# smups/rustronomy-watershed

Hardware: AMD Instinct MI355X
Metric: Mpixels/s segmenting watershed, 8192x8192 u8, device-resident (throughput, 4 transforms of distinct fields in flight; one transform alone: value_one_transform_alone) (higher is better)
Workload: dtype u8 image / u32 stamps+labels (integer min/max/compare); 1 GPU; 8192x8192 u8 uniform[0,254) random field per GPU, segmenting transform, max_water_level 254, seeds = find_local_minima (7320260 on rank 0's first field), engine fused; 4 contexts in flight, each transforming ITS OWN field and seed list (generator seeds 1..4); parallelism=independent fields x1, world_size=1, devices_visible=1, fields_per_gpu=1

## Files before the change

rustronomy-watershed_amd/csrc/ws_relax.hip:

```cpp
#include "ws_common.hpp"

#include <algorithm>
#include <cstdio>
#include <cstdlib>

namespace wsk {

typedef uint32_t u32x4_t __attribute__((ext_vector_type(4)));

#ifdef WS_DIAG_STAMPS
__device__ unsigned long long *g_diag = nullptr;
#define WS_STAMP(slot)                                                                          \
  do {                                                                                          \
    if (threadIdx.x == 0 && g_diag) g_diag[(size_t)blockIdx.x * 8 + (slot)] = __builtin_amdgcn_s_memrealtime(); \
  } while (0)
#define WS_STAMP_VALUE(slot, v)                                                                 \
  do {                                                                                          \
    if (threadIdx.x == 0 && g_diag) g_diag[(size_t)blockIdx.x * 8 + (slot)] = (v);              \
  } while (0)
#define WS_ACC_DECL unsigned long long ws_acc_t = 0, ws_acc[3] = {0, 0, 0}
#define WS_ACC_T0 (ws_acc_t = __builtin_amdgcn_s_memrealtime())
#define WS_ACC(k) do { const unsigned long long n_ = __builtin_amdgcn_s_memrealtime(); ws_acc[k] += n_ - ws_acc_t; ws_acc_t = n_; } while (0)
#define WS_ACC_STORE do { if (threadIdx.x == 0 && g_diag) { g_diag[(size_t)blockIdx.x * 8 + 5] = ws_acc[0]; g_diag[(size_t)blockIdx.x * 8 + 6] = ws_acc[1]; g_diag[(size_t)blockIdx.x * 8 + 7] = ws_acc[2]; } } while (0)
#else
// ... 1029 lines not shown
        run |= (st.x & ST_PASS) == pass || (st.y & ST_PASS) == pass || (st.z & ST_PASS) == pass || (st.w & ST_PASS) == pass;
      }
    run = run && tx * TW < W && ty * TH < H;
  }
  if ((uint32_t)t <= list_cap) tile_list[RL_HDR + 2 * (size_t)list_cap + t] = persist && run ? 1u : 0u;
  const unsigned long long todo = __builtin_amdgcn_ballot_w64(run);
  if (todo == 0) return;
  uint32_t base = 0;
  if (lane == 0) {
    base = atomicAdd(&tile_list[persist ? RLQ_TAIL : (pass & 3u)], (uint32_t)__popcll(todo));
    if (persist) atomicAdd(&tile_list[RLQ_PENDING], (uint32_t)__popcll(todo));
  }
  base = __shfl(base, 0, 64);
  const uint32_t idx = base + (uint32_t)__popcll(todo & ((1ull << lane) - 1ull));
  if (persist == 2) {
    uint32_t *avail = tile_list + pq_base(list_cap);
    if (lane == 0) atomicAdd(avail, (uint32_t)__popcll(todo));
    if ((lane & 31) == 0) (avail + PQ_HDR)[(first >> 5) + (lane >> 5)] = (uint32_t)(todo >> (lane & 32));
  } else if (run && persist) reinterpret_cast<unsigned long long *>(tile_list + RL_HDR)[idx] = ((unsigned long long)(idx + 1u) << 32) | (uint32_t)t;
  else if (run) tile_list[RL_HDR + (pass & 1u) * (size_t)list_cap + idx] = (uint32_t)t;
}

template <int TW, int TH>
__global__ __launch_bounds__(256) void k_relax_list_all(int H, int W, int tilesX, int tilesY, uint32_t pass, uint32_t *tile_list, uint32_t list_cap) {
  const int t = blockIdx.x * blockDim.x + threadIdx.x;
  if (t == 0) { tile_list[pass & 3u] = (uint32_t)(tilesX * tilesY); tile_list[4 + (pass & 3u)] = 0u; }
  if ((uint32_t)t <= list_cap) tile_list[RL_HDR + 2 * (size_t)list_cap + t] = 0u;
  if (t < tilesX * tilesY) tile_list[RL_HDR + (pass & 1u) * (size_t)list_cap + t] = (uint32_t)t;
}

size_t relax_list_words(int h, int w) {
  const uint32_t tiles = (uint32_t)relax_tiles(h, w);
  return pq_base(tiles) + PQ_HDR + (size_t)PQ_B * pq_words_per_bucket(tiles);
}

#ifndef WS_SPLIT_NW
#define WS_SPLIT_NW RX_NW
#endif
constexpr int RX_SNW = WS_SPLIT_NW;
constexpr int RX_STW = RX_TW / 2, RX_STH = 2 * RX_SNW * RX_P;
#ifndef WS_QUEUE_NW
#define WS_QUEUE_NW 16
#endif
constexpr int RX_QNW = WS_QUEUE_NW;
constexpr int RX_QTH = 2 * RX_QNW * RX_P;
size_t relax_tiles(int h, int w) {
  const int th = RX_NW * RX_P;
  const size_t a = (size_t)((w + RX_TW - 1) / RX_TW + 1) * ((h + th - 1) / th + 1);
  const size_t b = (size_t)((w + RX_STW - 1) / RX_STW + 1) * ((h + RX_STH - 1) / RX_STH + 1);
  return std::max(a, b);
}

__global__ void k_flag_tile_rows(uint32_t *prev, int sx, int bottom_row, uint32_t pass, int halo_flags) {
  const int i = blockIdx.x * blockDim.x + threadIdx.x;
  if (i >= sx * 4) return;
  if (halo_flags & 1) prev[i] = pass;
  if (halo_flags & 2) prev[(size_t)bottom_row * sx * 4 + i] = pass;
}

hipError_t block_flag_border_tiles(hipStream_t s, uint32_t *stamps, int h, int w, uint32_t pass, int halo_flags) {
  if ((pass & 1u) != 0 || h == 0 || w == 0) return hipErrorInvalidValue;
  const int th = RX_NW * RX_P;
  const int sx = (w + RX_TW - 1) / RX_TW + 1;
  const size_t cap = relax_tiles(h, w) * 4;
  const int bottom_row = (h - 2) / th + 1;
  k_flag_tile_rows<<<(sx * 4 + 255) / 256, 256, 0, s>>>(stamps + cap, sx, bottom_row, pass, halo_flags);
  return hipGetLastError();
}

constexpr int RX0_PH = 2 * RX_P;
constexpr int RX0_TH = RX_NW * RX0_PH;
typedef uint32_t tall_t[RX0_PH][RX_P];

template <bool TRACK, bool DOWN>
__device__ __forceinline__ void tall_sweep_rows(tall_t &T, const tall_t &B, const uint32_t (&up)[RX_P], const uint32_t (&dn)[RX_P],
                                                const uint32_t (&L)[RX0_PH], const uint32_t (&R)[RX0_PH], bool &changed) {
#pragma unroll
  for (int k = 0; k < RX0_PH; ++k) {
    const int r = DOWN ? k : RX0_PH - 1 - k;
#pragma unroll
    for (int c = 0; c < RX_P; ++c)
      relax_px<TRACK>(T[r][c], B[r][c], r == 0 ? up[c] : T[r - 1][c], r == RX0_PH - 1 ? dn[c] : T[r + 1][c],
                      c == 0 ? L[r] : T[r][c - 1], c == RX_P - 1 ? R[r] : T[r][c + 1], changed);
  }
}
template <bool TRACK, bool RIGHT>
__device__ __forceinline__ void tall_sweep_cols(tall_t &T, const tall_t &B, const uint32_t (&up)[RX_P], const uint32_t (&dn)[RX_P],
                                                const uint32_t (&L)[RX0_PH], const uint32_t (&R)[RX0_PH], bool &changed) {
#pragma unroll
  for (int k = 0; k < RX_P; ++k) {
    const int c = RIGHT ? k : RX_P - 1 - k;
#pragma unroll
    for (int r = 0; r < RX0_PH; ++r)
      relax_px<TRACK>(T[r][c], B[r][c], r == 0 ? up[c] : T[r - 1][c], r == RX0_PH - 1 ? dn[c] : T[r + 1][c],
                      c == 0 ? L[r] : T[r][c - 1], c == RX_P - 1 ? R[r] : T[r][c + 1], changed);
  }
}

__global__ __launch_bounds__(64 * RX_NW, 4) void k_relax0_tall(const uint8_t *__restrict__ img, uint32_t stride32, uint32_t *keys, int H, int W,
                                                               int tilesX, int flagAX, int flagSX, uint32_t max_level, uint32_t *stamps_own,
                                                               uint32_t *stamps_rerun, PassFlags pf, uint32_t max_iters,
                                                               const uint32_t *__restrict__ seed_mask, int SH, int check_carry, uint32_t *tile_list) {
  constexpr int NB = RX_NW, TW = RX_TW, TH = RX0_TH;
  constexpr uint32_t pass = 0;
  __shared__ __attribute__((aligned(16))) uint32_t sRow[2 * NB + 2][TW];
  __shared__ uint32_t s_flag[3];

  if (blockIdx.x == 0 && threadIdx.x < NSTRIPE)
    pf.edge_changed[((pass + 1) % COUNTER_RING) * FLAG_SLOT + threadIdx.x * STRIPE_STRIDE] = 0;
  if (tile_list && blockIdx.x == 0 && threadIdx.x == 0) { tile_list[(pass + 2) & 3u] = 0u; tile_list[4 + ((pass + 2) & 3u)] = 0u; }
  const int tile = (int)xcd_span_index(blockIdx.x, gridDim.x);
  const int tile_x = tile % tilesX, tile_y = tile / tilesX;
  const int x0 = tile_x * TW, y0 = tile_y * TH;
  if (x0 >= W || y0 >= H) return;
  const int tid = threadIdx.x, lane = tid & 63, band = tid >> 6;
  const int gx0 = x0 + lane * RX_P, gyb = y0 + band * RX0_PH;
  if (tid == 0) { s_flag[0] = 0; s_flag[1] = 0; s_flag[2] = 0; }

  tall_t T, B;
  uint32_t Lh[RX0_PH], Rh[RX0_PH];
  const bool dims24 = (uint32_t)W < (1u << 24) && (uint32_t)H < (1u << 24);
  const uint32_t gxc0 = (uint32_t)min(gx0, W - RX_P);
  const int xh_raw = lane < 32 ? x0 - 1 : x0 + TW;
  const uint32_t xh = (uint32_t)min(max(xh_raw, 0), W - 1);
  const bool xh_ok = lane < 32 ? x0 > 0 : x0 + TW < W;
  const int gy_halo_raw = band == 0 ? y0 - 1 : y0 + TH;
  const uint32_t gy_halo = (uint32_t)min(max(gy_halo_raw, 0), H - 1);
  u32x4_t halo_row;
  {
    uint32_t iv[RX0_PH];
#pragma unroll
    for (int r = 0; r < RX0_PH; ++r) {
      const uint32_t gyc = (uint32_t)min(gyb + r, H - 1);
      const uint32_t ro = dims24 ? __umul24(gyc, (uint32_t)W) : gyc * (uint32_t)W;
      const uint32_t p = ro + gxc0, ph_ = ro + xh;
      const uint32_t nib = seed_mask[p >> 5] >> (p & 31u);
      iv[r] = *reinterpret_cast<const uint32_t *>(img + ((unsigned long long)gyc * stride32 + gxc0));
      Lh[r] = (seed_mask[ph_ >> 5] >> (ph_ & 31u)) & 1u;
      T[r][0] = nib & 1u; T[r][1] = nib & 2u; T[r][2] = nib & 4u; T[r][3] = nib & 8u;
    }
    const uint32_t p = (dims24 ? __umul24(gy_halo, (uint32_t)W) : gy_halo * (uint32_t)W) + gxc0;
    const uint32_t nib = seed_mask[p >> 5] >> (p & 31u);
    halo_row = u32x4_t{nib & 1u, nib & 2u, nib & 4u, nib & 8u};
    if (max_level == 254u) {
#pragma unroll
      for (int r = 0; r < RX0_PH; ++r) {
        B[r][0] = (iv[r] << 24) | 1u;
        B[r][1] = ((iv[r] << 16) & 0xFF000000u) | 1u;
        B[r][2] = ((iv[r] << 8) & 0xFF000000u) | 1u;
        B[r][3] = (iv[r] & 0xFF000000u) | 1u;
      }
    } else {
#pragma unroll
      for (int r = 0; r < RX0_PH; ++r)
#pragma unroll
        for (int c = 0; c < RX_P; ++c) {
          const uint32_t v = (iv[r] >> (8 * c)) & 0xFFu;
          B[r][c] = v <= max_level ? ((v << 24) | 1u) : KEY_INF;
        }
    }
  }
#pragma unroll
  for (int r = 0; r < RX0_PH; ++r) {
#pragma unroll
    for (int c = 0; c < RX_P; ++c) T[r][c] = T[r][c] ? 0u : KEY_INF;
    Lh[r] = Lh[r] ? 0u : KEY_INF;
  }
  halo_row.x = halo_row.x ? 0u : KEY_INF; halo_row.y = halo_row.y ? 0u : KEY_INF;
  halo_row.z = halo_row.z ? 0u : KEY_INF; halo_row.w = halo_row.w ? 0u : KEY_INF;
  const bool inner = SH == H && x0 >= 1 && x0 + TW <= W - 1 && y0 >= 1 && y0 + TH <= H - 1;
  if (!inner) {
    int ry = SH == H ? gyb : gyb % SH;
#pragma unroll
    for (int r = 0; r < RX0_PH; ++r) {
      const int gy = gyb + r;
      const bool row_ok = gy < H, row_int = ry >= 1 && ry < SH - 1 && gy < H;
#pragma unroll
      for (int c = 0; c < RX_P; ++c) {
        const int gx = gx0 + c;
        if (!(row_ok && gx < W)) T[r][c] = KEY_INF;
        if (!(row_int && gx >= 1 && gx < W - 1)) B[r][c] = KEY_INF;
      }
      if (!(row_ok && xh_ok)) Lh[r] = KEY_INF;
      if (++ry == SH) ry = 0;
    }
    const bool ok = gy_halo_raw >= 0 && gy_halo_raw < H;
    if (!(ok && gx0 + 0 < W)) halo_row.x = KEY_INF;
    if (!(ok && gx0 + 1 < W)) halo_row.y = KEY_INF;
    if (!(ok && gx0 + 2 < W)) halo_row.z = KEY_INF;
    if (!(ok && gx0 + 3 < W)) halo_row.w = KEY_INF;
  }
#pragma unroll
  for (int r = 0; r < RX0_PH; ++r) {
#pragma unroll
    for (int c = 0; c < RX_P; ++c) B[r][c] = min(B[r][c], T[r][c]);
    Rh[r] = Lh[r];
  }
  auto refresh_columns = [&]() {
#pragma unroll
    for (int r = 0; r < RX0_PH; ++r) {
      Lh[r] = lane_left(Lh[r], T[r][3]);
      Rh[r] = lane_right(Rh[r], T[r][0]);
    }
  };
  auto publish_rows = [&]() {
    *reinterpret_cast<u32x4_t *>(&sRow[1 + 2 * band][lane * RX_P]) = u32x4_t{T[0][0], T[0][1], T[0][2], T[0][3]};
    *reinterpret_cast<u32x4_t *>(&sRow[2 + 2 * band][lane * RX_P]) = u32x4_t{T[RX0_PH - 1][0], T[RX0_PH - 1][1], T[RX0_PH - 1][2], T[RX0_PH - 1][3]};
  };
  if (band == 0) *reinterpret_cast<u32x4_t *>(&sRow[0][lane * RX_P]) = halo_row;
  if (band == NB - 1) *reinterpret_cast<u32x4_t *>(&sRow[2 * NB + 1][lane * RX_P]) = halo_row;
  publish_rows();
  __syncthreads();

  uint32_t iters = 0;
  bool unfinished = max_iters == 0;
  uint32_t up[RX_P], dn[RX_P];
  auto fetch_rows = [&]() {
    const u32x4_t up4 = *reinterpret_cast<const u32x4_t *>(&sRow[2 * band][lane * RX_P]);
    const u32x4_t dn4 = *reinterpret_cast<const u32x4_t *>(&sRow[2 * band + 3][lane * RX_P]);
    up[0] = up4.x; up[1] = up4.y; up[2] = up4.z; up[3] = up4.w;
    dn[0] = dn4.x; dn[1] = dn4.y; dn[2] = dn4.z; dn[3] = dn4.w;
  };
  for (; max_iters != 0;) {
    ++iters;
    if (iters <= 2) {
      bool untracked = false;
      fetch_rows();
      refresh_columns();
      tall_sweep_rows<false, true>(T, B, up, dn, Lh, Rh, untracked);
      refresh_columns();
      tall_sweep_cols<false, true>(T, B, up, dn, Lh, Rh, untracked);
      refresh_columns();
      tall_sweep_rows<false, false>(T, B, up, dn, Lh, Rh, untracked);
      publish_rows();
      __syncthreads();
    }
    bool changed = false;
    fetch_rows();
    refresh_columns();
    tall_sweep_cols<true, false>(T, B, up, dn, Lh, Rh, changed);
    const uint32_t slot = (iters - 1) % 3;
    if (__builtin_amdgcn_ballot_w64(changed) != 0) {
      publish_rows();
      if (lane == 0) s_flag[slot] = 1;
    }
    __syncthreads();
    const bool again = s_flag[slot] != 0;
    if (tid == 0) s_flag[(slot + 2) % 3] = 0;
    if (!again) break;
    if (iters >= max_iters) { unfinished = true; break; }
  }

  uint32_t ovf = 0;
  if (gx0 < W) {
#pragma unroll
    for (int r = 0; r < RX0_PH; ++r) {
      const int gy = gyb + r;
      if (gy < H) *reinterpret_cast<u32x4_t *>(keys + (size_t)gy * W + gx0) = u32x4_t{T[r][0], T[r][1], T[r][2], T[r][3]};
      if (check_carry) {
#pragma unroll
        for (int c = 0; c < RX_P; ++c)
          ovf |= (T[r][c] != 0u && T[r][c] < KEY_INF && (T[r][c] & RING_MASK) == 0u);
      }
    }
  }
  if (ovf) atomicExch(pf.overflow, 1u);
  const uint32_t stripe = (blockIdx.x % NSTRIPE) * STRIPE_STRIDE;
  auto matters = [](uint32_t now, uint32_t across) { return now != 0u && now + 1u < across; };
  bool edge = false;
  if (band == 0) {
    const u32x4_t a = *reinterpret_cast<const u32x4_t *>(&sRow[0][lane * RX_P]);
    edge |= matters(T[0][0], a.x) || matters(T[0][1], a.y) || matters(T[0][2], a.z) || matters(T[0][3], a.w);
  }
  if (band == NB - 1) {
    const u32x4_t a = *reinterpret_cast<const u32x4_t *>(&sRow[2 * NB + 1][lane * RX_P]);
    constexpr int l = RX0_PH - 1;
    edge |= matters(T[l][0], a.x) || matters(T[l][1], a.y) || matters(T[l][2], a.z) || matters(T[l][3], a.w);
  }
  if (lane == 0 || lane == 63) {
#pragma unroll
    for (int r = 0; r < RX0_PH; ++r) edge |= matters(T[r][lane == 0 ? 0 : 3], lane == 0 ? Lh[r] : Rh[r]);
  }
  if (edge) pf.edge_changed[(pass % COUNTER_RING) * FLAG_SLOT + stripe] = 1u;
  if (tid == 0) {
    if (unfinished) {
#pragma unroll
      for (int k = 0; k < RX0_TH / (RX_NW * RX_P); ++k) {
        const int fy = tile_y * (RX0_TH / (RX_NW * RX_P)) + k;
        if (fy * (RX_NW * RX_P) >= H) break;
        stamps_rerun[((size_t)fy * flagSX + tile_x + 1) * 4 + 2] = pass + 2;
        uint32_t *own = stamps_own + ((size_t)fy * flagAX + tile_x) * 4;
        own[0] = pass + 1; own[1] = pass + 1; own[2] = pass + 1; own[3] = pass + 1;
      }
      pf.edge_changed[(pass % COUNTER_RING) * FLAG_SLOT + stripe] = 1u;
    }
    pf.any_change[stripe] = 1u;
    if (pf.stats) {
      atomicAdd(&pf.stats[stripe], (uint32_t)(TW * TH / 2048));
      atomicAdd(&pf.stats[FLAG_SLOT + stripe], 2u * iters);
    }
  }
}

bool relax_uses_seam_repair(int h, int w, bool seed_bits, int slice_h, bool padded, size_t seam_min_px) {
  const int ax = (w + RX_TW - 1) / RX_TW, ay = (h + RX_NW * RX_P - 1) / (RX_NW * RX_P);
  (void)slice_h;
  return seed_bits && !padded && (w & 3) == 0 && ax >= 2 && ay >= 2 && (size_t)h * (size_t)w >= seam_min_px;
}

hipError_t relax_pass(hipStream_t s, const uint8_t *img, size_t img_stride, uint32_t *keys, int h, int w,
                      uint32_t max_level, uint32_t pass, uint32_t *stamps, PassFlags pf, uint32_t max_iters,
                      const uint32_t *seed_labels, bool seed_bits, int slice_h, bool carry_checked_later, bool padded,
                      uint32_t *tile_list, size_t seam_min_px, int persistent_pass) {
  const int th = RX_NW * RX_P;
  const int pad = padded ? 1 : 0;
  const int check_carry = carry_checked_later ? 0 : 1;
  const int sh = slice_h > 0 ? slice_h : h;
  const int ax = (w + RX_TW - 1) / RX_TW, ay = (h + th - 1) / th;
  const int sx = ax + 1, sy = ay + 1;
  static const uint32_t same_from_passes = [] {
    const char *e = tuning_env("WS_RELAX_SAME_GRID_FROM");
    const uint32_t v = e ? (uint32_t)atoi(e) : RX_SAME_GRID_FROM;
    return v < 3u ? 3u : (v | 1u);
  }();
  static const uint32_t queue_from = [] {
    const char *e = tuning_env("WS_RELAX_QUEUE_FROM");
    const uint32_t v = e ? (uint32_t)atoi(e) : 3u;
    return v < 3u ? 3u : (v | 1u);
  }();
  const int persist_mode = tuning_env("WS_RELAX_PERSIST") ? atoi(tuning_env("WS_RELAX_PERSIST")) : persistent_pass;
  const bool queue_plane = persist_mode == 2 && tile_list && !pad && (w & 3) == 0 && w >= RX_P &&
                           ((reinterpret_cast<uintptr_t>(img) | img_stride) & 3u) == 0 && relax_tiles(h, w) < (1u << 24);
  const bool early_queue = (queue_plane || (persist_mode == 4 && tile_list)) && queue_from < same_from_passes;
  const uint32_t same_from = early_queue ? queue_from : same_from_passes;
  const int read_same = pass >= same_from ? 1 : 0, write_same = pass + 1 >= same_from ? 1 : 0;
  const uint32_t list_cap = (uint32_t)relax_tiles(h, w);
  const int shifted = read_same ? 0 : (int)(pass & 1u);
  const int tx = shifted ? sx : ax, ty = shifted ? sy : ay;
  const size_t cap = relax_tiles(h, w) * 4;
  const uint32_t *prev = stamps + ((pass + 1) & 1) * cap;
  uint32_t *cur = stamps + (pass & 1) * cap;
  const int ox_ = read_same ? ax : (shifted ? ax : sx), oy_ = read_same ? ay : (shifted ? ay : sy);
  static const uint32_t p0_rounds = [] {
    const char *e = tuning_env("WS_RELAX_P0_ROUNDS");
    return e ? (uint32_t)atoi(e) : 2u;
  }();
  static const bool no_seam = tuning_env("WS_RELAX_NO_SEAM") != nullptr;
  const bool seam_flow = !no_seam && seed_labels != nullptr && relax_uses_seam_repair(h, w, seed_bits, slice_h, padded, seam_min_px);
  constexpr uint32_t SEAM_P0_ROUNDS = 6;
  const uint32_t p0_cap = seam_flow ? SEAM_P0_ROUNDS : p0_rounds;
  if (pass == 0 && p0_cap < max_iters) max_iters = p0_cap;
  static const uint32_t late_cap = [] {
    const char *e = tuning_env("WS_RELAX_LATE_CAP");
    return e ? (uint32_t)atoi(e) : RX_LATE_ROUND_CAP;
  }();
  static const uint32_t scan_from_knob = [] {
    const char *e = tuning_env("WS_RELAX_SCAN_FROM");
    return e ? (uint32_t)atoi(e) : RX_SCAN_FROM_PASS;
  }();
  const uint32_t scan_from = early_queue ? same_from - 1u : std::max(scan_from_knob, 1u);
  if (pass >= scan_from && late_cap != 0 && late_cap < max_iters) max_iters = late_cap;
  if (const char *e = tuning_env("WS_RELAX_WIDE_CAP")) {
    int n_ = 0, c_ = 0;
    if (sscanf(e, "%d,%d", &n_, &c_) == 2 && pass >= scan_from && pass < scan_from + (uint32_t)n_) max_iters = (uint32_t)c_;
  }
  static const uint32_t early_cap = [] {
    const char *e = tuning_env("WS_RELAX_EARLY_CAP");
    return e ? (uint32_t)atoi(e) : RX_EARLY_ROUND_CAP;
  }();
  if (pass >= 1 && pass < scan_from && early_cap != 0 && early_cap < max_iters) max_iters = early_cap;
  static const uint32_t lite_from = [] {
    const char *e = tuning_env("WS_RELAX_LITE_FROM");
    return e ? (uint32_t)atoi(e) : 2u;
  }();
  static const uint32_t chunk_from = [] {
    const char *e = tuning_env("WS_RELAX_CHUNK_FROM");
    return e ? (uint32_t)atoi(e) : 3u;
  }();
  constexpr uint32_t SEAM_REPAIR_ROUNDS = 4;
  static const int seam_band = [] { const char *e = tuning_env("WS_RELAX_SEAM_BAND"); return e ? atoi(e) : 6; }();
  static const bool no_tall = tuning_env("WS_RELAX_NO_TALL") != nullptr;
  const bool tall0 = seam_flow && !no_tall && seam_band == 6 && h > RX0_TH && w >= RX_P &&
                     ((reinterpret_cast<uintptr_t>(img) | img_stride) & 3u) == 0 && img_stride <= 0xFFFFFFFFull;
  const int ay_tall = (h + RX0_TH - 1) / RX0_TH;
  if (tall0 && pass == 0) {
    k_relax0_tall<<<ax * ay_tall, 64 * RX_NW, 0, s>>>(img, (uint32_t)img_stride, keys, h, w, ax, ax, sx, max_level, cur, const_cast<uint32_t *>(prev), pf,
                                                     max_iters, seed_labels, sh, check_carry, tile_list);
    return hipGetLastError();
  }
  if (tall0 && pass == 1) {
    k_relax<3, false, false, false, false, 1, 0, RX0_TH><<<ax * (ay_tall - 1), 192, 0, s>>>(img, img_stride, keys, h, w, ax, ay_tall - 1, sx, sy, 0, 1, max_level, pass, prev, cur,
                                                                                          pf, SEAM_REPAIR_ROUNDS, nullptr, 0, sh, check_carry, pad, tile_list, 0, 0, 0, list_cap, 0);
  } else if (seam_flow && pass == 1) {
    if (seam_band == 4)
      k_relax<2, false, false, false, false, 1><<<ax * (ay - 1), 128, 0, s>>>(img, img_stride, keys, h, w, ax, ay - 1, sx, sy, 0, 1, max_level, pass, prev, cur,
                                                                            pf, SEAM_REPAIR_ROUNDS, nullptr, 0, sh, check_carry, pad, tile_list, 0, 0, 0, list_cap, 0);
    else if (seam_band == 6)
      k_relax<3, false, false, false, false, 1><<<ax * (ay - 1), 192, 0, s>>>(img, img_stride, keys, h, w, ax, ay - 1, sx, sy, 0, 1, max_level, pass, prev, cur,
                                                                            pf, SEAM_REPAIR_ROUNDS, nullptr, 0, sh, check_carry, pad, tile_list, 0, 0, 0, list_cap, 0);
    else
      k_relax<4, false, false, false, false, 1><<<ax * (ay - 1), 256, 0, s>>>(img, img_stride, keys, h, w, ax, ay - 1, sx, sy, 0, 1, max_level, pass, prev, cur,
                                                                            pf, SEAM_REPAIR_ROUNDS, nullptr, 0, sh, check_carry, pad, tile_list, 0, 0, 0, list_cap, 0);
  }
  if (seam_flow && pass == 1) {
    hipError_t e = hipGetLastError();
    if (e != hipSuccess) return e;
    const int strips_x = (ax - 1 + 31) / 32;
    k_relax<RX_NW, false, false, false, false, 2><<<strips_x * ay, 64 * RX_NW, 0, s>>>(img, img_stride, keys, h, w, strips_x, ay, sx, sy, 0, 1, max_level, pass,
                                                                                       prev, cur, pf, SEAM_REPAIR_ROUNDS, nullptr, 0, sh, check_carry, pad, tile_list, 0, 0,
                                                                                       0, list_cap, 0);
    return hipGetLastError();
  }
  const int sb = pass == 0 && seed_labels && seed_bits ? 1 : 0;
  const uint32_t *sl = pass == 0 ? seed_labels : nullptr;
  const uint32_t chunk_from_now = seam_flow ? std::min(chunk_from, 2u) : chunk_from;
  if (pass < chunk_from_now && pass < lite_from) {
    k_relax<RX_NW, false, false, false><<<tx * ty, 64 * RX_NW, 0, s>>>(img, img_stride, keys, h, w, tx, ty, ox_, oy_, shifted, seam_flow && pass == 0 ? 3 : 1, max_level, pass,
                                                                       prev, cur, pf, max_iters, sl, sb, sh, check_carry, pad, tile_list, 0, read_same, write_same, list_cap, 0);
  } else if (pass < chunk_from_now) {
    k_relax<RX_NW, false, false, true><<<tx * ty, 64 * RX_NW, 0, s>>>(img, img_stride, keys, h, w, tx, ty, ox_, oy_, shifted, 1, max_level, pass,
                                                                      prev, cur, pf, max_iters, sl, sb, sh, check_carry, pad, tile_list, 0, read_same, write_same, list_cap, 0);
  } else {
    const int chunk = 4;
    const unsigned grid = (unsigned)((tx * ty + chunk - 1) / chunk);
    static const uint32_t list_from_passes = [] {
      const char *e = tuning_env("WS_RELAX_LIST_FROM");
      return e ? (uint32_t)atoi(e) : RX_LIST_FROM_PASS;
    }();
    const uint32_t list_from = early_queue ? same_from : list_from_passes;
    if (pass < scan_from) {
      k_relax<RX_NW, true, false, true><<<grid, 64 * RX_NW, 0, s>>>(img, img_stride, keys, h, w, tx, ty, ox_, oy_, shifted, chunk, max_level,
                                                              pass, prev, cur, pf, max_iters, nullptr, 0, sh, check_carry, pad, tile_list, 0, read_same, write_same, list_cap, 0);
    } else if (tile_list && pass >= list_from && pass >= scan_from + 1) {
      static const bool no_append = tuning_env("WS_RELAX_NO_APPEND") != nullptr;
      const uint32_t first_list_pass = std::max(list_from, scan_from + 1);
      const int append_next = !no_append && pass >= same_from && pass >= first_list_pass ? 1 : 0;
      const bool appended = !no_append && pass >= 1 && pass - 1 >= same_from && pass - 1 >= first_list_pass;
      static const bool no_split = tuning_env("WS_RELAX_NO_SPLIT") != nullptr;
      const bool split = !no_split && pass >= same_from && same_from >= first_list_pass;
      const int gx = split ? (w + RX_STW - 1) / RX_STW : tx, gy = split ? (h + RX_STH - 1) / RX_STH : ty;
      if (!appended) {
        const unsigned blocks = (unsigned)((std::max<size_t>((size_t)gx * gy, list_cap + 1) + 255) / 256);
        const bool persist = (persist_mode == 1 || persist_mode == 2) && split && pass == same_from && !pad && (w & 3) == 0 && w >= RX_P &&
                             ((reinterpret_cast<uintptr_t>(img) | img_stride) & 3u) == 0 && (size_t)gx * gy <= list_cap && list_cap < (1u << 24);
        if (persist) {
          const bool in_order = persist_mode == 2;
          hipError_t e = hipMemsetAsync(tile_list + RL_HDR, 0, 2 * (size_t)list_cap * sizeof(uint32_t), s);
          if (e == hipSuccess) e = hipMemsetAsync(tile_list + 8, 0, (RL_HDR - 8) * sizeof(uint32_t), s);
          if (e == hipSuccess && in_order)
            e = hipMemsetAsync(tile_list + pq_base(list_cap), 0, (PQ_HDR + (size_t)PQ_B * pq_words_per_bucket(list_cap)) * sizeof(uint32_t), s);
          if (e != hipSuccess) return e;
          const int qy = (h + RX_QTH - 1) / RX_QTH;
          if (in_order)
            k_relax_list_regrid<RX_STW, RX_QTH, RX_TW, RX_NW * RX_P><<<blocks, 256, 0, s>>>(h, w, gx, qy, ax, ay, pass, prev, tile_list, list_cap, 2);
          else
            k_relax_list_regrid<RX_STW, RX_STH, RX_TW, RX_NW * RX_P><<<blocks, 256, 0, s>>>(h, w, gx, gy, ax, ay, pass, prev, tile_list, list_cap, 1);
          if ((e = hipGetLastError()) != hipSuccess) return e;
          const unsigned workers = tuning_env("WS_RELAX_PERSIST_WORKERS") ? (unsigned)atoi(tuning_env("WS_RELAX_PERSIST_WORKERS"))
                                                                          : std::min<unsigned>(in_order ? RX_LIST_GRID / 2 : RX_LIST_GRID * RX_NW / RX_SNW, (unsigned)(gx * (in_order ? qy : gy)));
          const uint32_t cap = tuning_env("WS_RELAX_PERSIST_CAP") ? (uint32_t)atoi(tuning_env("WS_RELAX_PERSIST_CAP")) : RLQ_ROUND_CAP;
          const int mode = tuning_env("WS_RELAX_PERSIST_MODE") ? atoi(tuning_env("WS_RELAX_PERSIST_MODE")) : 0;
          if (in_order)
            k_relax<RX_QNW, true, true, true, true, 0, 2><<<workers, 64 * RX_QNW, 0, s>>>(img, img_stride, keys, h, w, gx, qy, gx, qy, 0, chunk, max_level, pass, prev, cur, pf, cap,
                                                                                         nullptr, 0, sh, check_carry, pad, tile_list, mode, 1, 1, list_cap, 1);
          else
            k_relax<RX_SNW, true, true, true, true, 0, 1><<<workers, 64 * RX_SNW, 0, s>>>(img, img_stride, keys, h, w, gx, gy, gx, gy, 0, chunk, max_level, pass, prev, cur, pf, cap,
                                                                                         nullptr, 0, sh, check_carry, pad, tile_list, mode, 1, 1, list_cap, 1);
          if ((e = hipGetLastError()) != hipSuccess) return e;
          hipStreamCaptureStatus capturing = hipStreamCaptureStatusNone;
          (void)hipStreamIsCapturing(s, &capturing);
          if (tuning_env("WS_RELAX_PERSIST_DIAG") && capturing == hipStreamCaptureStatusNone) {
            uint32_t hd[RL_HDR];
            (void)hipStreamSynchronize(s);
            (void)hipMemcpy(hd, tile_list, sizeof hd, hipMemcpyDeviceToHost);
            fprintf(stderr, "[ws] persistent pass %u: pushed %u popped %u pending %u done %u runs %u | workers wait %.1f us, life %.1f us (sums / 512), polls %u\n", pass,
                    hd[RLQ_TAIL], hd[RLQ_HEAD], hd[RLQ_PENDING], hd[RLQ_DONE], hd[RLQ_RUNS], hd[RLQ_WAIT] / 100.0 / 512.0, hd[RLQ_LIFE] / 100.0 / 512.0, hd[RLQ_POLLS]);
            const double runs = hd[RLQ_RUNS] ? hd[RLQ_RUNS] : 1;
            fprintf(stderr, "[ws]   per tile run (us): load %.2f rounds %.2f epilogue %.2f hand-in %.2f; shader clock %.0f MHz\n", hd[RLQ_PHASE] / 100.0 / runs, hd[RLQ_PHASE + 1] / 100.0 / runs,
                    hd[RLQ_PHASE + 2] / 100.0 / runs, hd[RLQ_PHASE + 3] / 100.0 / runs, hd[RLQ_LIFE] ? 256.0 * hd[RLQ_PHASE + 4] / hd[RLQ_LIFE] * 100.0 : 0.0);
          }
          k_relax_list_all<RX_STW, RX_STH><<<(unsigned)((std::max<size_t>((size_t)gx * gy, list_cap + 1) + 255) / 256), 256, 0, s>>>(h, w, gx, gy, pass + 1, tile_list, list_cap);
          return hipGetLastError();
        }
        if (split && pass == same_from)
          k_relax_list_regrid<RX_STW, RX_STH, RX_TW, RX_NW * RX_P><<<blocks, 256, 0, s>>>(h, w, gx, gy, ax, ay, pass, prev, tile_list, list_cap, 0);
        else if (split)
          k_relax_list<RX_STW, RX_STH><<<blocks, 256, 0, s>>>(h, w, gx, gy, gx, gy, 0, pass, prev, tile_list, 1, list_cap);
        else
          k_relax_list<RX_TW, RX_NW * RX_P><<<blocks, 256, 0, s>>>(h, w, tx, ty, ox_, oy_, shifted, pass, prev, tile_list, read_same, list_cap);
        hipError_t e = hipGetLastError();
        if (e != hipSuccess) return e;
      }
      if (split)
        k_relax<RX_SNW, true, true, true, true><<<std::min<unsigned>(RX_LIST_GRID * RX_NW / RX_SNW, (unsigned)(gx * gy)), 64 * RX_SNW, 0, s>>>(
            img, img_stride, keys, h, w, gx, gy, gx, gy, 0, chunk, max_level, pass, prev, cur, pf, max_iters, nullptr, 0, sh,
            check_carry, pad, tile_list, 1, 1, 1, list_cap, append_next);
      else
        k_relax<RX_NW, true, true, true><<<std::min<unsigned>(RX_LIST_GRID, (unsigned)(tx * ty)), 64 * RX_NW, 0, s>>>(
            img, img_stride, keys, h, w, tx, ty, ox_, oy_, shifted, chunk, max_level, pass, prev, cur, pf, max_iters, nullptr, 0, sh,
            check_carry, pad, tile_list, 1, read_same, write_same, list_cap, append_next);
    } else {
      k_relax<RX_NW, true, true, true><<<grid, 64 * RX_NW, 0, s>>>(img, img_stride, keys, h, w, tx, ty, ox_, oy_, shifted, chunk, max_level,
                                                             pass, prev, cur, pf, max_iters, nullptr, 0, sh, check_carry, pad, tile_list, 0, read_same, write_same, list_cap, 0);
    }
  }
  return hipGetLastError();
}

}
```

Before: 160,300 Mpixels/s.

## Add tall-tile vertical seam strip relaxation kernel for pass one

Adds a specialized kernel that relaxes the vertical seams between column tiles using tall tiles (RX0_TH rows) held in registers, with DPP lane exchange for horizontal neighbours and shared-memory row exchange between bands. It replaces the generic strip kernel when the tall pass-0 layout is active, covering each seam with fewer, taller blocks. Blocks whose seam stamps are already settled exit early, and stamp marking follows the tall-tile geometry. It adds a new code path with its own boundary and stamp logic, which can be disabled through an environment variable.

```diff
diff --git a/rustronomy-watershed_amd/csrc/ws_relax.hip b/rustronomy-watershed_amd/csrc/ws_relax.hip
--- a/rustronomy-watershed_amd/csrc/ws_relax.hip
+++ b/rustronomy-watershed_amd/csrc/ws_relax.hip
@@ -1355,6 +1355,239 @@
   }
 }
 
+__global__ __launch_bounds__(64 * RX_NW, 4) void k_relax_strips_tall(const uint8_t *__restrict__ img, uint32_t stride32, uint32_t *keys, int H, int W,
+                                                                     int stripsX, int flagSX, uint32_t max_level, uint32_t pass, uint32_t *stamps_cur,
+                                                                     PassFlags pf, uint32_t max_iters, int SH, int check_carry, uint32_t *tile_list) {
+  constexpr int NB = RX_NW, TW = RX_TW, TH = RX0_TH;
+  constexpr int SEAM_PY = RX_NW * RX_P, SEAM_PX = RX_TW;
+  __shared__ __attribute__((aligned(16))) uint32_t sRow[2 * NB + 2][TW];
+  __shared__ __attribute__((aligned(16))) uint32_t sInitRow[2][TW];
+  __shared__ uint32_t s_flag[3];
+  __shared__ uint32_t s_edges;
+  __shared__ uint64_t s_sum[64 * NB];
+  __shared__ uint32_t sInitCol[RX0_PH][64 * NB];
+
+  if (blockIdx.x == 0 && threadIdx.x < NSTRIPE)
+    pf.edge_changed[((pass + 1) % COUNTER_RING) * FLAG_SLOT + threadIdx.x * STRIPE_STRIDE] = 0;
+  if (tile_list && blockIdx.x == 0 && threadIdx.x == 0) { tile_list[(pass + 2) & 3u] = 0u; tile_list[4 + ((pass + 2) & 3u)] = 0u; }
+  const int tile = (int)xcd_span_index(blockIdx.x, gridDim.x);
+  const int tile_x = tile % stripsX, tile_y = tile / stripsX;
+  const int y0 = tile_y * TH;
+  if (y0 >= H || (tile_x * 32 + 1) * SEAM_PX >= W) return;
+  const int tid = threadIdx.x, lane = tid & 63, band = tid >> 6;
+  const int seam_x = (tile_x * 32 + (lane >> 1) + 1) * SEAM_PX;
+  const bool has_seam = seam_x < W;
+  const int fx = seam_x / SEAM_PX - 1 + (lane & 1);
+  {
+    bool settled = true;
+#pragma unroll
+    for (int k = 0; k < TH / SEAM_PY; ++k) {
+      const int fy = tile_y * (TH / SEAM_PY) + k;
+      const bool there = has_seam && fy * SEAM_PY < H;
+      const uint32_t word = stamps_cur[there ? ((size_t)fy * flagSX + fx + 1) * 4 + 2 : 2];
+      settled &= !there || word == pass + 1;
+    }
+    if (__builtin_amdgcn_ballot_w64(settled) == ~0ull) return;
+  }
+  const int gx0 = has_seam ? seam_x - RX_P + (lane & 1) * RX_P : W, gyb = y0 + band * RX0_PH;
+  if (tid == 0) { s_edges = 0; s_flag[0] = 0; s_flag[1] = 0; s_flag[2] = 0; }
+
+  tall_t T, B;
+  uint32_t halo[RX0_PH];
+  const uint32_t gxc0 = (uint32_t)min(gx0, W - RX_P);
+  const int xh_raw = (lane & 1) ? gx0 + RX_P : gx0 - 1;
+  const uint32_t xh = (uint32_t)min(max(xh_raw, 0), W - 1);
+  const bool xh_ok = has_seam && xh_raw < W;
+  const int gy_halo_raw = band == 0 ? y0 - 1 : y0 + TH;
+  const uint32_t gy_halo = (uint32_t)min(max(gy_halo_raw, 0), H - 1);
+  u32x4_t halo_row;
+  {
+    u32x4_t kv[RX0_PH];
+    uint32_t iv[RX0_PH];
+#pragma unroll
+    for (int r = 0; r < RX0_PH; ++r) {
+      const uint32_t gyc = (uint32_t)min(gyb + r, H - 1);
+      iv[r] = *reinterpret_cast<const uint32_t *>(img + ((unsigned long long)gyc * stride32 + gxc0));
+      kv[r] = *reinterpret_cast<const u32x4_t *>(keys + (size_t)gyc * W + gxc0);
+      halo[r] = keys[(size_t)gyc * W + xh];
+    }
+    halo_row = *reinterpret_cast<const u32x4_t *>(keys + (size_t)gy_halo * W + gxc0);
+#pragma unroll
+    for (int r = 0; r < RX0_PH; ++r) { T[r][0] = kv[r].x; T[r][1] = kv[r].y; T[r][2] = kv[r].z; T[r][3] = kv[r].w; }
+    if (max_level == 254u) {
+#pragma unroll
+      for (int r = 0; r < RX0_PH; ++r) {
+        B[r][0] = (iv[r] << 24) | 1u;
+        B[r][1] = ((iv[r] << 16) & 0xFF000000u) | 1u;
+        B[r][2] = ((iv[r] << 8) & 0xFF000000u) | 1u;
+        B[r][3] = (iv[r] & 0xFF000000u) | 1u;
+      }
+    } else {
+#pragma unroll
+      for (int r = 0; r < RX0_PH; ++r)
+#pragma unroll
+        for (int c = 0; c < RX_P; ++c) {
+          const uint32_t v = (iv[r] >> (8 * c)) & 0xFFu;
+          B[r][c] = v <= max_level ? ((v << 24) | 1u) : KEY_INF;
+        }
+    }
+  }
+  {
+    int ry = SH == H ? gyb : gyb % SH;
+#pragma unroll
+    for (int r = 0; r < RX0_PH; ++r) {
+      const int gy = gyb + r;
+      const bool row_ok = gy < H, row_int = ry >= 1 && ry < SH - 1 && gy < H;
+#pragma unroll
+      for (int c = 0; c < RX_P; ++c) {
+        const int gx = gx0 + c;
+        if (!(row_ok && gx < W)) T[r][c] = KEY_INF;
+        if (!(row_int && gx >= 1 && gx < W - 1)) B[r][c] = KEY_INF;
+      }
+      if (!(row_ok && xh_ok)) halo[r] = KEY_INF;
+      if (++ry == SH) ry = 0;
+    }
+    const bool ok = gy_halo_raw >= 0 && gy_halo_raw < H;
+    if (!(ok && gx0 + 0 < W)) halo_row.x = KEY_INF;
+    if (!(ok && gx0 + 1 < W)) halo_row.y = KEY_INF;
+    if (!(ok && gx0 + 2 < W)) halo_row.z = KEY_INF;
+    if (!(ok && gx0 + 3 < W)) halo_row.w = KEY_INF;
+  }
+  uint32_t Lh[RX0_PH], Rh[RX0_PH];
+  {
+    uint64_t sum_before = 0;
+#pragma unroll
+    for (int r = 0; r < RX0_PH; ++r) {
+#pragma unroll
+      for (int c = 0; c < RX_P; ++c) {
+        B[r][c] = min(B[r][c], T[r][c]);
+        sum_before += T[r][c];
+      }
+      Lh[r] = halo[r];
+      Rh[r] = halo[r];
+      sInitCol[r][tid] = (lane & 1) ? T[r][RX_P - 1] : T[r][0];
+    }
+    s_sum[tid] = sum_before;
+  }
+  auto refresh_columns = [&]() {
+#pragma unroll
+    for (int r = 0; r < RX0_PH; ++r) {
+      Lh[r] = lane_left(Lh[r], T[r][RX_P - 1]);
+      Rh[r] = lane_right(Rh[r], T[r][0]);
+      Lh[r] = (lane & 1) ? Lh[r] : halo[r];
+      Rh[r] = (lane & 1) ? halo[r] : Rh[r];
+    }
+  };
+  auto publish_rows = [&]() {
+    *reinterpret_cast<u32x4_t *>(&sRow[1 + 2 * band][lane * RX_P]) = u32x4_t{T[0][0], T[0][1], T[0][2], T[0][3]};
+    *reinterpret_cast<u32x4_t *>(&sRow[2 + 2 * band][lane * RX_P]) = u32x4_t{T[RX0_PH - 1][0], T[RX0_PH - 1][1], T[RX0_PH - 1][2], T[RX0_PH - 1][3]};
+  };
+  if (band == 0) {
+    *reinterpret_cast<u32x4_t *>(&sRow[0][lane * RX_P]) = halo_row;
+    *reinterpret_cast<u32x4_t *>(&sInitRow[0][lane * RX_P]) = u32x4_t{T[0][0], T[0][1], T[0][2], T[0][3]};
+  }
+  if (band == NB - 1) {
+    *reinterpret_cast<u32x4_t *>(&sRow[2 * NB + 1][lane * RX_P]) = halo_row;
+    *reinterpret_cast<u32x4_t *>(&sInitRow[1][lane * RX_P]) = u32x4_t{T[RX0_PH - 1][0], T[RX0_PH - 1][1], T[RX0_PH - 1][2], T[RX0_PH - 1][3]};
+  }
+  publish_rows();
+  __syncthreads();
+
+  uint32_t iters = 0;
+  bool unfinished = max_iters == 0;
+  uint32_t up[RX_P], dn[RX_P];
+  auto fetch_rows = [&]() {
+    const u32x4_t up4 = *reinterpret_cast<const u32x4_t *>(&sRow[2 * band][lane * RX_P]);
+    const u32x4_t dn4 = *reinterpret_cast<const u32x4_t *>(&sRow[2 * band + 3][lane * RX_P]);
+    up[0] = up4.x; up[1] = up4.y; up[2] = up4.z; up[3] = up4.w;
+    dn[0] = dn4.x; dn[1] = dn4.y; dn[2] = dn4.z; dn[3] = dn4.w;
+  };
+  for (; max_iters != 0;) {
+    ++iters;
+    {
+      bool untracked = false;
+      fetch_rows();
+      refresh_columns();
+      tall_sweep_rows<false, true>(T, B, up, dn, Lh, Rh, untracked);
+      refresh_columns();
+      tall_sweep_cols<false, true>(T, B, up, dn, Lh, Rh, untracked);
+      refresh_columns();
+      tall_sweep_rows<false, false>(T, B, up, dn, Lh, Rh, untracked);
+      publish_rows();
+      __syncthreads();
+    }
+    bool changed = false;
+    fetch_rows();
+    refresh_columns();
+    tall_sweep_cols<true, false>(T, B, up, dn, Lh, Rh, changed);
+    const uint32_t slot = (iters - 1) % 3;
+    if (__builtin_amdgcn_ballot_w64(changed) != 0) {
+      publish_rows();
+      if (lane == 0) s_flag[slot] = 1;
+    }
+    __syncthreads();
+    const bool again = s_flag[slot] != 0;
+    if (tid == 0) s_flag[(slot + 2) % 3] = 0;
+    if (!again) break;
+    if (iters >= max_iters) { unfinished = true; break; }
+  }
+
+  uint64_t sum_after = 0;
+#pragma unroll
+  for (int r = 0; r < RX0_PH; ++r)
+#pragma unroll
+    for (int c = 0; c < RX_P; ++c) sum_after += T[r][c];
+  uint32_t e = 0, ovf = 0;
+  if (has_seam && sum_after != s_sum[tid]) {
+#pragma unroll
+    for (int r = 0; r < RX0_PH; ++r) {
+      const int gy = gyb + r;
+      if (gy < H) *reinterpret_cast<u32x4_t *>(keys + (size_t)gy * W + gx0) = u32x4_t{T[r][0], T[r][1], T[r][2], T[r][3]};
+      if (check_carry) {
+#pragma unroll
+        for (int c = 0; c < RX_P; ++c)
+          ovf |= (T[r][c] != 0u && T[r][c] < KEY_INF && (T[r][c] & RING_MASK) == 0u);
+      }
+    }
+    e |= 16u;
+  }
+  if (ovf) atomicExch(pf.overflow, 1u);
+  auto matters = [](uint32_t before, uint32_t now, uint32_t across) { return before != now && now + 1u < across; };
+  if (has_seam) {
+    const uint32_t mark = pass + 1;
+    bool col = unfinished;
+#pragma unroll
+    for (int r = 0; r < RX0_PH; ++r) col |= matters(sInitCol[r][tid], (lane & 1) ? T[r][RX_P - 1] : T[r][0], halo[r]);
+    bool top = false, bottom = false;
+    if (band == 0) {
+      const u32x4_t o = *reinterpret_cast<const u32x4_t *>(&sInitRow[0][lane * RX_P]);
+      const u32x4_t a = *reinterpret_cast<const u32x4_t *>(&sRow[0][lane * RX_P]);
+      top = matters(o.x, T[0][0], a.x) || matters(o.y, T[0][1], a.y) || matters(o.z, T[0][2], a.z) || matters(o.w, T[0][3], a.w);
+    }
+    if (band == NB - 1) {
+      const u32x4_t o = *reinterpret_cast<const u32x4_t *>(&sInitRow[1][lane * RX_P]);
+      const u32x4_t a = *reinterpret_cast<const u32x4_t *>(&sRow[2 * NB + 1][lane * RX_P]);
+      constexpr int l = RX0_PH - 1;
+      bottom = matters(o.x, T[l][0], a.x) || matters(o.y, T[l][1], a.y) || matters(o.z, T[l][2], a.z) || matters(o.w, T[l][3], a.w);
+    }
+    if (col && gyb < H) { stamps_cur[((size_t)(gyb / SEAM_PY) * flagSX + fx) * 4 + 3] = mark; e |= 1u; }
+    if (top && y0 > 0) { stamps_cur[((size_t)((y0 - 1) / SEAM_PY) * flagSX + fx) * 4 + 3] = mark; e |= 1u; }
+    if (bottom && y0 + TH < H) { stamps_cur[((size_t)((y0 + TH) / SEAM_PY) * flagSX + fx) * 4 + 3] = mark; e |= 1u; }
+  }
+  if (e) atomicOr(&s_edges, e);
+  __syncthreads();
+  if (tid == 0) {
+    const uint32_t ed = s_edges;
+    const uint32_t stripe = (blockIdx.x % NSTRIPE) * STRIPE_STRIDE;
+    if (ed & 1u) pf.edge_changed[(pass % COUNTER_RING) * FLAG_SLOT + stripe] = 1u;
+    if (ed) pf.any_change[stripe] = 1u;
+    if (pf.stats) {
+      atomicAdd(&pf.stats[stripe], (uint32_t)(TW * TH / 2048));
+      atomicAdd(&pf.stats[FLAG_SLOT + stripe], 2u * iters);
+    }
+  }
+}
+
 bool relax_uses_seam_repair(int h, int w, bool seed_bits, int slice_h, bool padded, size_t seam_min_px) {
   const int ax = (w + RX_TW - 1) / RX_TW, ay = (h + RX_NW * RX_P - 1) / (RX_NW * RX_P);
   (void)slice_h;
@@ -1459,6 +1692,12 @@
     hipError_t e = hipGetLastError();
     if (e != hipSuccess) return e;
     const int strips_x = (ax - 1 + 31) / 32;
+    static const bool no_tall_strips = tuning_env("WS_RELAX_NO_TALL_STRIPS") != nullptr;
+    if (tall0 && !no_tall_strips) {
+      k_relax_strips_tall<<<strips_x * ay_tall, 64 * RX_NW, 0, s>>>(img, (uint32_t)img_stride, keys, h, w, strips_x, sx, max_level, pass, cur, pf,
+                                                                  SEAM_REPAIR_ROUNDS, sh, check_carry, tile_list);
+      return hipGetLastError();
+    }
     k_relax<RX_NW, false, false, false, false, 2><<<strips_x * ay, 64 * RX_NW, 0, s>>>(img, img_stride, keys, h, w, strips_x, ay, sx, sy, 0, 1, max_level, pass,
                                                                                        prev, cur, pf, SEAM_REPAIR_ROUNDS, nullptr, 0, sh, check_carry, pad, tile_list, 0, 0,
                                                                                        0, list_cap, 0);
```

Measured after the change: 165,200 Mpixels/s (median of 6 runs). +3.1%, better.
